# narayanan2004/GraphMat

Hardware: AMD Instinct MI355X
Metric: GTEPS (edges/s) per iter + achieved HBM GB/s, PageRank RMAT-26 (higher is better)
Workload: dtype f32

## Files before the change

graphmat_amd/csrc/gm_programs.hip:

```cpp
#include <limits.h>
#include <math.h>

#include <string>

#include "GraphMatRuntime.h"
#include "gm_internal.hpp"

#define HD __host__ __device__

namespace gm {

extern int g_short_row, g_giant_row, g_rank_by, g_rank_cap, g_col_tiles, g_tile_min_row, g_long_mid, g_tile_balance, g_own_wave_row, g_sort_tile_lists, g_sweep_slices, g_sweep_acc_limit, g_sweep_long_limit, g_sweep_long_row, g_sweep_fold_share, g_sweep_border_factor, g_blocked_rows, g_sweep_waves, g_sweep_stream, g_sweep_stream_weight;
static int g_force_ordered = 0;

struct PRv : gm_pr_t {
  HD PRv() { pagerank = 0.3; degree = 0; }
  HD int operator!=(const PRv& p) { return ((double)fabsf(p.pagerank - pagerank) > 1e-5); }
};

struct DegreeP : GraphMat::GraphProgram<int, int, PRv, int> {
  DegreeP() {
    this->order = GraphMat::IN_EDGES;
    this->process_message_requires_vertexprop = false;
  }
// ... 600 lines not shown

void warm_program_kernels(void* d_scratch256) {
  static bool done = false;
  if (done || !d_scratch256) return;
  done = true;
  hipLaunchKernelGGL(GraphMat::dev::k_fill_u32, dim3(1), dim3(GraphMat::dev::kBlock), 0, 0, (uint32_t*)d_scratch256, (int64_t)64, 0u);
  (void)hipDeviceSynchronize();
}

}

extern "C" {

namespace gm {
struct EngineKey { const char* name; int index; int def, lo, hi; };
static const EngineKey kEngineKeys[] = {
  {"debug_flags", 0, 0, 0, 0x7fffffff},
  {"wave16_form", 1, 2, 0, 31},
  {"rowwave_form", 2, 4, 0, 31},
  {"persist_per_cu", 3, 0, 0, 8},
  {"giant_maps", 4, 1, 0, 1},
  {"ordered_giant_two_pass", 5, 2, 0, 2},
  {"fuse_apply_send", 6, 1, 0, 1},
  {"untiled_pass_plain", 7, 1, 0, 1},
  {"last_rows_lanes", 8, 8, 8, 16},
  {"push_edge_permille", 9, 50, 0, 1000},
  {"bits_step_edges", 10, 2 << 20, 0, 0x7fffffff},
  {"sparse_step_edges", 11, 1 << 20, 0, 0x7fffffff},
  {"iteration_trace", 12, 0, 0, 1},
  {"ablate_cold_from", 13, 0, 0, 0x7fffffff},
  {"ablate_cold_short", 14, 0, 0, 0x7fffffff},
  {"two_stage_head_permille", 15, 900, 100, 990},
  {"giant_stream", 16, 1, 0, 2},
  {"sweep_form", 17, 0, 0, 511},
  {"blocked_form", 18, 2, 0, 31},
  {"guided_pull", 19, 1, 0, 2},
};
static_assert(offsetof(gm_engine_options_t, guided_pull) == 19 * sizeof(int32_t), "kEngineKeys follows the field order");
static bool engine_value_ok(const EngineKey& k, int v) {
  if (v < k.lo || v > k.hi) return false;
#ifndef GRAPHMAT_ABLATION
  if (!strcmp(k.name, "debug_flags") && (v & (15 | 16384)) != 0) return false;
  if (!strncmp(k.name, "ablate_", 7)) return false;
#endif
  if (!strcmp(k.name, "wave16_form")) return (v & 15) <= 5;
  if (!strcmp(k.name, "rowwave_form")) return (v & 15) <= 4;
  if (!strcmp(k.name, "last_rows_lanes")) return v == 8 || v == 16;
  return true;
}
static gm_engine_options_t engine_documented_defaults() {
  gm_engine_options_t o;
  memset(&o, 0, sizeof(o));
  for (const EngineKey& k : kEngineKeys) ((int32_t*)&o)[k.index] = k.def;
  const char* tr = getenv("GRAPHMAT_ITERATION_TRACE");
  if (tr && tr[0] == '1') o.iteration_trace = 1;
  if (const char* env = getenv("GRAPHMAT_OPTIONS")) {
    std::string all(env);
    size_t pos = 0;
    while (pos < all.size()) {
      size_t end = all.find(',', pos);
      if (end == std::string::npos) end = all.size();
      const std::string kv = all.substr(pos, end - pos);
      pos = end + 1;
      const size_t eq = kv.find('=');
      bool ok = false;
      if (eq != std::string::npos) {
        const std::string key = kv.substr(0, eq);
// ... 193 lines not shown
```

include/graphmat/engine.hpp:

```cpp
#pragma once
#include <stdio.h>
#include <stdlib.h>
#include <sys/time.h>

#include <limits>
#include <type_traits>
#include <vector>

#include "kernels.hpp"

namespace GraphMat {

enum edge_direction { OUT_EDGES, IN_EDGES, ALL_EDGES };
enum activity_type { ACTIVE_ONLY, ALL_VERTICES };

template <class T, class U, class V, class E>
class GraphProgram;

namespace detail {

template <class F>
struct member_class_of;
template <class C, class R, class... A>
struct member_class_of<R (C::*)(A...)> { typedef C type; };
// ... 784 lines not shown
        list_ready = frontier_v <= (unsigned long long)dev::kSparseListCap;
      }
    }
    if (xsparse_candidate) {
      int still = xsparse_ok ? 1 : 0;
      gm_graph_exchange(g, GM_XCHG_CONVERGED, nullptr, 0, nullptr, &still);
      if (!still) xsparse_ok = false;
    }
    if (xsparse_ok) {
      int dummy = 0;
      exchange_state(&dummy);
    }
    if (act == ALL_VERTICES) fill_active();
    timer = PhaseTimer(gm_graph_timing_enabled(g) != 0, s);
    tick("first frontier counted", (int)frontier_v);
    if (!(opt.debug_flags & dev::DBG_NO_OVERLAP)) {
      aux.attach(res_stream, res_fork, res_join);
    }
    if constexpr (program_row_filter<P>::enabled) {
      void* pw = nullptr;
      if (gm_graph_workspace(g, 8, ((size_t)(n + 31) / 32 + 2) * 4, &pw) == GM_OK) {
        d_want = (uint32_t*)pw;
        dev::ProgArg<P> pa0 = dev::make_prog_arg(gp);
        hipLaunchKernelGGL((dev::k_want_init<P, V>), dim3(grid_for(n_live)), dim3(dev::kBlock), 0, s, pa0, (const V*)d_vp, n_live, d_want);
      }
    }
    grouped_waves = !(opt.debug_flags & dev::DBG_NO_GROUPED);
  }

  void finish(int it) {
    GM_HIP_OK(hipStreamSynchronize(s));
    gm_graph_note_set(g, 3, (int64_t)sparse_sweeps);
    gm_graph_note_set(g, 4, (int64_t)short_folds);
    tick("loop done", it);
    aux.finish();
    st.iterations = it;
    timer.finish(&st);
    gm_graph_record_stats(g, &st);
    tick("teardown done", 0);
  }

  bool two_stage_applies() const {
    if (!(multi && act == ALL_VERTICES && order == OUT_EDGES && iterations > 0 && !(opt.debug_flags & dev::DBG_NO_PIPELINE) && !trace && inherits_iteration_hook<P>()))
      return false;
    if constexpr (sizeof(T) == 4 && sizeof(U) == 4 && std::is_trivially_copyable<T>::value && std::is_trivially_copyable<U>::value) {
      gm_sweep_t sw;
      if (!use_vp && gm_graph_sweep(g, &sw) == GM_OK && sw.nslices > 1 && desc.nshards > 1 && !(opt.debug_flags & (dev::DBG_NO_TILES | dev::DBG_NO_OVERLAP))) return false;
    }
    return true;
  }
  int run_two_stage() {
    void* x2v = nullptr;
    size_t x2_bytes = 0;
    int x2_ext = 0;
    int32_t rs = 0, bs = 0, ms = 0;
    bool staged = false;
    bool have_x2 = gm_graph_workspace_info(g, 9, &x2v, &x2_bytes, &x2_ext) == GM_OK && x2_ext && x2v != nullptr && x2_bytes >= (size_t)desc.ndevice * sizeof(T);
    if (!have_x2 && gm_graph_exchange_is_native(g))
      have_x2 = gm_graph_workspace(g, 9, (size_t)desc.ndevice * sizeof(T) + 64, &x2v) == GM_OK && x2v != nullptr;
    if (have_x2) {
      int64_t agreed = 0;
      if (gm_graph_note_get(g, 0, &agreed) == GM_OK) {
        rs = (int32_t)agreed;
        staged = rs > 0 && gm_graph_split(g, GM_DIR_OUT, opt.two_stage_head_permille, &rs, &bs, &ms) == GM_OK;
      } else {
        int mine = (gm_graph_split(g, GM_DIR_OUT, opt.two_stage_head_permille, &rs, &bs, &ms) == GM_OK) ? -rs : 0;
// ... 352 lines not shown
            hipLaunchKernelGGL((dev::k_spmv_sell_w12<P, T, U, V, E, false>), dim3(256), dim3(768), 0, s, pa, set, stage, sw.nslices, sw.nrows_long, sw.slice_base, sw.scol,
                               (const uint32_t*)nullptr, sw.wrow, sw.row_of_slot, sw.lcol, (const uint32_t*)nullptr, sw.lps, sw.lrow_of_slot, sw.gcol,
                               (const uint32_t*)nullptr, sw.gdst, sw.gslice, gt, xq, y);
          continue;
        }
        if (sterms != nullptr && set == 0) {
          if constexpr (sizeof(E) == 4 && std::is_trivially_copyable<E>::value) {
            if (Aout.vals != nullptr) {
              hipLaunchKernelGGL((dev::k_spmv_sell_stream<P, T, U, V, E, true>), dim3(256), dim3(1024), 0, s, pa, set, stage, sw.nslices, sw.nrows_long, sw.slice_base, sw.scol,
                                 sw.sval, sw.wrow_stream, sw.row_of_slot, sw.lcol, sw.lval, sw.lps, sw.lrow_of_slot, sw.gcol, sw.gval, sw.gdst, sw.gslice, gt, xq, y, sterms);
              with_vals = true;
            }
          }
          if (!with_vals)
            hipLaunchKernelGGL((dev::k_spmv_sell_stream<P, T, U, V, E, false>), dim3(256), dim3(1024), 0, s, pa, set, stage, sw.nslices, sw.nrows_long, sw.slice_base, sw.scol,
                               (const uint32_t*)nullptr, sw.wrow_stream, sw.row_of_slot, sw.lcol, (const uint32_t*)nullptr, sw.lps, sw.lrow_of_slot, sw.gcol,
                               (const uint32_t*)nullptr, sw.gdst, sw.gslice, gt, xq, y, sterms);
          continue;
        }
        if constexpr (sizeof(E) == 4 && std::is_trivially_copyable<E>::value) {
          if (Aout.vals != nullptr) {
            hipLaunchKernelGGL((dev::k_spmv_sell<P, T, U, V, E, true>), dim3(256), dim3(1024), 0, s, pa, set, stage, sw.nslices, sw.nrows_long, sw.slice_base, sw.scol,
                               sw.sval, sw.wrow, sw.row_of_slot, sw.lcol, sw.lval, sw.lps, sw.lrow_of_slot, sw.gcol, sw.gval, sw.gdst, sw.gslice, gt, xq, y);
            with_vals = true;
          }
        }
        if (!with_vals)
          hipLaunchKernelGGL((dev::k_spmv_sell<P, T, U, V, E, false>), dim3(256), dim3(1024), 0, s, pa, set, stage, sw.nslices, sw.nrows_long, sw.slice_base, sw.scol,
                             (const uint32_t*)nullptr, sw.wrow, sw.row_of_slot, sw.lcol, (const uint32_t*)nullptr, sw.lps, sw.lrow_of_slot, sw.gcol,
                             (const uint32_t*)nullptr, sw.gdst, sw.gslice, gt, xq, y);
      }
      st.spmv_launches += sw.nsets;
      timer.mark(TAG_WAVE);
      if (gterms != nullptr && !chain_done) {
        GM_HIP_OK(hipEventRecord(aux.fork, s));
        GM_HIP_OK(hipStreamWaitEvent(aux.s, aux.fork, 0));
        if (gather_apart) giant_gather();
        Launch Lg = L;
        Lg.terms_ready = true;
        launch_spmv_vp<P, T, U, V, E>(use_vp, Lg, pa, Ag, xq, xb, (const V*)d_vp, y, ybits, acc, rk);
      }
      if (where == 2) short_rows();
      if (where == 4) {
        hipLaunchKernelGGL((dev::k_short_fold<P, U>), dim3((unsigned)sw.nbins), dim3(512), 0, s, pa, (const U*)sterms, sw.sinv, sw.schunk, sw.nslices, sw.bin_cap, sw.sbin_row,
                           sw.soff, sw.srow, y, (acc & dev::ACC_STATIC_BITS) ? (uint32_t*)nullptr : ybits);
        st.spmv_launches++;
        short_folds++;
        if (verbose && !said_short_fold) { printf("GraphMat(HIP):   the rows of up to %d edges ride the sweep (k_short_fold)\n", (int)sw.short_row); said_short_fold = true; }
        timer.mark(TAG_ROWBLOCK);
      }
      if (aux.pending && !defer_join) GM_HIP_OK(hipStreamWaitEvent(s, aux.join, 0));
      aux.keep = aux.forked = aux.pending = false;
      timer.mark(defer_join ? TAG_ROWBLOCK : TAG_GIANT);
      if (shorts_blocked) {
        launch_blocked(pa, bl);
        st.spmv_launches += 1;
        timer.mark(TAG_ROWBLOCK);
      }
      if (!defer_join) check_probed(pa, Aout, xb != nullptr ? (const uint32_t*)ybits : Aout.rowbits, nullptr, acc, ybits, xb == nullptr);
    } else {
      (void)pa; (void)acc; (void)sw; (void)defer_join;
    }
  }

  bool swept_pipeline_applies(gm_sweep_t* sw) {
    if constexpr (kSparseT && sizeof(T) == 4 && sizeof(U) == 4 && std::is_trivially_copyable<U>::value) {
      if (!(multi && act == ALL_VERTICES && order == OUT_EDGES && iterations > 1 && !(opt.debug_flags & dev::DBG_NO_PIPELINE) && !trace && inherits_iteration_hook<P>())) return false;
      if (!(gm_graph_exchange_caps(g) & GM_XCAP_SPARSE) || rk_unverified || opt.fuse_apply_send == 0) return false;
      xq = x;
      xb = nullptr;
      int fine = (sweep_usable(dev::ACC_STATIC_BITS, sw) && sw->nsub > 1 && Aout.ngiant <= dev::kSparseListCap && n_live >= 64) ? 1 : 0;
      gm_graph_exchange(g, GM_XCHG_CONVERGED, nullptr, 0, nullptr, &fine);
      return fine == 1;
    } else {
      (void)sw;
      return false;
    }
  }
  int run_swept_sharded(const gm_sweep_t& sw) {
    if constexpr (kSparseT && sizeof(T) == 4 && sizeof(U) == 4 && std::is_trivially_copyable<U>::value) {
      void* x2v = nullptr;
// ... 55 lines not shown
          timer.mark(TAG_SEND);
          aux.wait_join(s);
          timer.mark(TAG_GIANT);
          hipLaunchKernelGGL((dev::k_apply_send_list<P, T, U, V>), dim3(grid_for(cap)), dim3(dev::kBlock), 0, s, pa, (const U*)y, (const uint32_t*)bits_giant, d_vp, d_active,
                             Aout.giant_row, Aout.ngiant, d_changed, xnext, desc.row_lo, gather + (size_t)desc.shard * cap, cap);
          timer.mark(TAG_APPLY);
          int hf[2] = {cap, 0};
          if (gm_graph_exchange(g, GM_XCHG_GATHER, gather, (int64_t)sizeof(xentry_t), nullptr, hf) != 0) die("giant rows' message exchange failed");
          if (gm_graph_exchange(g, GM_XCHG_WAIT, xnext, (int64_t)sizeof(T), nullptr, nullptr) != 0) die("message exchange wait failed");
          const int64_t nall = (int64_t)desc.nshards * cap;
          hipLaunchKernelGGL((dev::k_unpack_frontier<T>), dim3(grid_for(nall)), dim3(dev::kBlock), 0, s, (const xentry_t*)gather, nall, xnext, xbits);
          timer.mark(TAG_SEND);
        } else {
          hipLaunchKernelGGL((dev::k_apply<P, U, V, false>), dim3(ag), dim3(dev::kBlock), 0, s, pa, (const U*)y, Aout.rowbits, d_vp, d_active, n_live, d_changed,
                             (const int64_t*)nullptr, (unsigned long long*)nullptr, (uint32_t*)nullptr, (int32_t*)nullptr, (unsigned int*)nullptr);
          timer.mark(TAG_APPLY);
        }
        if (n_live < n && it == 0) GM_HIP_OK(hipMemsetAsync(d_active + n_live / 32, 0, (size_t)(nwords - n_live / 32) * 4, s));
        gp->do_every_iteration(it);
        T* t = xcur; xcur = xnext; xnext = t;
      }
      fill_active();
      finish(it);
      return it;
    } else {
      (void)sw;
      return -1;
    }
  }

  bool said_blocked = false, said_sparse_sweep = false, said_short_fold = false;
  int sparse_sweeps = 0;
  int short_folds = 0;
  bool blocked_usable(int acc, gm_blocked_t* bl) {
    if constexpr (sizeof(T) == 4 && sizeof(U) == 4 && std::is_trivially_copyable<T>::value && std::is_trivially_copyable<U>::value) {
      if (use_vp || xq == nullptr || xb != nullptr || d_want != nullptr || program_row_filter<P>::enabled || (acc & dev::ACC_READ_PREV)) return false;
      if (!(rk == REDUCE_ORDERED || rk == REDUCE_F32_ADD || rk == REDUCE_COMMUTATIVE)) return false;
      if (opt.debug_flags & dev::DBG_NO_TILES) return false;
      if (gm_graph_blocked(g, bl) != GM_OK || bl->nrows <= 0 || bl->short_row != Aout.short_row) return false;
      if (Aout.vals != nullptr && !(bl->val_bytes == 4 && bl->eval != nullptr && sizeof(E) == 4 && std::is_trivially_copyable<E>::value)) return false;
      return true;
    } else {
      (void)acc; (void)bl;
      return false;
    }
  }
  void launch_blocked(const dev::ProgArg<P>& pa, const gm_blocked_t& bl) {
    if constexpr (sizeof(T) == 4 && sizeof(U) == 4 && std::is_trivially_copyable<T>::value && std::is_trivially_copyable<U>::value) {
      static int cus_of[64] = {0};
      constexpr bool kValsOk = sizeof(E) == 4 && std::is_trivially_copyable<E>::value;
      int dev_id = 0;
      GM_HIP_OK(hipGetDevice(&dev_id));
      int& cus = cus_of[dev_id & 63];
      if (cus == 0) {
        GM_HIP_OK(hipFuncSetAttribute((const void*)&dev::k_spmv_blocked<P, T, U, V, E, false, 2>, hipFuncAttributeMaxDynamicSharedMemorySize, GM_BLOCKED_ROWS * 4));
        GM_HIP_OK(hipFuncSetAttribute((const void*)&dev::k_spmv_blocked<P, T, U, V, E, false, 4>, hipFuncAttributeMaxDynamicSharedMemorySize, GM_BLOCKED_ROWS * 4));
        if constexpr (kValsOk) {
          GM_HIP_OK(hipFuncSetAttribute((const void*)&dev::k_spmv_blocked<P, T, U, V, E, true, 2>, hipFuncAttributeMaxDynamicSharedMemorySize, GM_BLOCKED_ROWS * 4));
          GM_HIP_OK(hipFuncSetAttribute((const void*)&dev::k_spmv_blocked<P, T, U, V, E, true, 4>, hipFuncAttributeMaxDynamicSharedMemorySize, GM_BLOCKED_ROWS * 4));
        }
        int n = 0;
        GM_HIP_OK(hipDeviceGetAttribute(&n, hipDeviceAttributeMultiprocessorCount, dev_id));
        cus = n > 0 ? n : 1;
      }
      if (verbose && !said_blocked) { printf("GraphMat(HIP):   the short rows take the column-blocked stream (%d rows, %lld edges%s)\n", bl.nrows, (long long)bl.nentries, Aout.vals ? ", with their edge values" : ""); said_blocked = true; }
      static int fits_of[64] = {0};
// ... 121 lines not shown
        const int nf = (int)frontier_v;
        const unsigned pieces = (unsigned)(frontier_e / dev::kPieceEdges + frontier_v);
        piece_offsets(nf);
        hipLaunchKernelGGL(dev::k_mark_rows_of_list, dim3(pieces > 0 ? pieces : 1), dim3(dev::kBlock), 0, s, Asrc, (const int32_t*)d_list, nf, (const unsigned int*)d_off, d_mark);
      } else {
        const int mgrid = grid_for(n_live) < 4096 ? grid_for(n_live) : 4096;
        hipLaunchKernelGGL(dev::k_mark_rows_of_active, dim3(mgrid), dim3(dev::kBlock), 0, s, Asrc, (const uint32_t*)d_active, n_live, d_mark);
      }
      row_bits = d_mark;
      guided_few = frontier_e <= 4096ull;
      if (verbose) printf("GraphMat(HIP):   guided pull: %llu active vertices, %llu out-edges\n", frontier_v, frontier_e);
    }
    if (dense_push) {
      multiply_dense_push(pa);
    } else if (order == OUT_EDGES || order == ALL_EDGES) {
      const int acc = static_bits ? dev::ACC_STATIC_BITS : 0;
      const uint32_t* xsum = nullptr;
      const unsigned long long present_x = xsparse_ok ? (unsigned long long)xs_total : frontier_v;
      if (want_stats && rk == REDUCE_LAST && xb != nullptr && present_x * 512ull < (unsigned long long)n_live * (unsigned long long)desc.nshards) {
        void* ps = nullptr;
        const int xwords = (desc.ndevice + 31) / 32;
        const int nsum = (xwords / 2 + 31) / 32 + 1;
        if (gm_graph_workspace(g, 11, (size_t)nsum * 4 + 64, &ps) == GM_OK) {
          hipLaunchKernelGGL(dev::k_bits_summary, dim3(grid_for(nsum)), dim3(dev::kBlock), 0, s, xb, xwords, (uint32_t*)ps, nsum);
          xsum = (const uint32_t*)ps;
        }
      }
      int ntile = 1;
      if (dense_x && !multi && row_bits == nullptr && rk != REDUCE_LAST && dev::stageable<T>::value && !(opt.debug_flags & dev::DBG_NO_TILES))
        gm_graph_tiles(g, GM_DIR_OUT, &ntile);
      gm_sweep_t sw;
      gm_blocked_t bl;
      if (row_bits == nullptr && !xsp && sweep_usable(acc, &sw)) {
        multiply_out_swept(pa, acc, sw);
      } else if (dense_x && !multi && row_bits == nullptr && blocked_usable(acc, &bl)) {
        multiply_out_blocked(pa, acc, bl);
      } else if (ntile > 1) {
        multiply_out_tiled(pa, ntile, acc);
      } else {
        launch_spmv_vp<P, T, U, V, E>(use_vp, launch_ctx(), pa, Aout, xq, xb, (const V*)d_vp, y, ybits, acc, rk, row_bits, grouped_waves && guided_few, xsum);
        check_probed(pa, Aout, static_bits ? Aout.rowbits : (const uint32_t*)ybits, row_bits, acc, ybits, dense_x);
      }
      if (static_bits) apply_bits = Aout.rowbits;
    }
    if (!dense_push && (order == IN_EDGES || order == ALL_EDGES)) {
      int acc = (order == ALL_EDGES) ? dev::ACC_READ_PREV : 0;
      uint32_t* yb = ybits;
      if (static_bits) {
        acc |= dev::ACC_STATIC_BITS;
        yb = const_cast<uint32_t*>(Aout.rowbits);
        apply_bits = Ain.rowbits;
        if (order == ALL_EDGES && gm_graph_rowbits_all(g, &apply_bits) != GM_OK) die(gm_last_error());
      }
      launch_spmv_vp<P, T, U, V, E>(use_vp, launch_ctx(), pa, Ain, (const T*)x, xb, (const V*)d_vp, y, yb, acc, rk, (const uint32_t*)d_want, grouped_waves);
      if (order == IN_EDGES) check_probed(pa, Ain, static_bits ? Ain.rowbits : (const uint32_t*)ybits, d_want, acc, ybits, dense_x);
    }
    lap("SPMV time");
    if (trace) tr_updated = count_bits(apply_bits, n_live);
    const bool build_list = want_stats && frontier_e <= (4ull << 20);
    if (want_stats) GM_HIP_OK(hipMemsetAsync(d_count, 0, 4, s));
    listed = build_list;
    const int apply_cap = build_list ? dev::kApplyMaxBlocks / 4 : dev::kApplyMaxBlocks;
    const int apply_grid = grid_for(n_live) < apply_cap ? grid_for(n_live) : apply_cap;
    if (want_stats)
      hipLaunchKernelGGL((dev::k_apply<P, U, V, true>), dim3(apply_grid), dim3(dev::kBlock), 0, s, pa, (const U*)y, apply_bits, d_vp, d_active, n_live,
                         d_changed, Asrc.rowptr, d_striped, d_want, build_list ? d_list : (int32_t*)nullptr, build_list ? d_count : (unsigned int*)nullptr);
    else if (inherits_iteration_hook<P>() && dense_x && !lazy_send && !trace && opt.fuse_apply_send != 0 && iterations > 0 && it + 1 < iterations) {
      hipLaunchKernelGGL((dev::k_apply_send<P, T, U, V>), dim3(apply_grid), dim3(dev::kBlock), 0, s, pa, (const U*)y, apply_bits, d_vp, d_active, n_live,
                         d_changed, d_want, x, xbits, desc.row_lo);
      x_presend = true;
    } else
      hipLaunchKernelGGL((dev::k_apply<P, U, V, false>), dim3(apply_grid), dim3(dev::kBlock), 0, s, pa, (const U*)y, apply_bits, d_vp, d_active, n_live,
                         d_changed, (const int64_t*)nullptr, (unsigned long long*)nullptr, d_want, (int32_t*)nullptr, (unsigned int*)nullptr);
    if (n_live < n && it == 0)
      GM_HIP_OK(hipMemsetAsync(d_active + n_live / 32, 0, (size_t)(nwords - n_live / 32) * 4, s));
    timer.mark(TAG_APPLY);
    lap("Apply time");
  }

  int run_loop() {
    int it = 0;
    tick("setup done", 0);
    while (true) {
      tick("iteration", it);
      if (trace) { (void)hipStreamSynchronize(s); gettimeofday(&tr_iter, 0); tr_last = tr_iter; }
      tr_updated = -1;
      if (verbose && can_push) printf("GraphMat(HIP):   active set: %llu vertices, %llu out-edges (max %llu)\n", frontier_v, frontier_e, frontier_maxdeg);
      dev::ProgArg<P> pa = dev::make_prog_arg(gp);
      const bool want_stats = (can_push || xsparse_ok || guided) && iterations <= 0;
      if (iterations <= 0) GM_HIP_OK(hipMemsetAsync(d_changed, 0, want_stats ? sizeof(int) + striped_bytes : sizeof(int), s));
      timer.mark(TAG_START);
      const bool xsp = xsparse_ok && xs_max <= dev::kSparseListCap &&
                       (unsigned long long)xs_max * sizeof(xentry_t) * 2ull < (unsigned long long)n_live * sizeof(T);
      const bool push = can_push && frontier_v > 0 && frontier_v <= (unsigned long long)dev::kSparseListCap &&
                        frontier_e * 1000ull < (unsigned long long)Aout.nnz * (unsigned long long)opt.push_edge_permille;
      const bool sparse = push && frontier_e <= (unsigned long long)opt.sparse_step_edges;
      const bool dense_push = push && !sparse && rk == REDUCE_LAST;
// ... 56 lines not shown
```

include/graphmat/kernels.hpp:

```cpp
#pragma once
#include <hip/hip_runtime.h>
#include <stdint.h>
#include <string.h>

#include <type_traits>

#include "../graphmat_hip.h"

namespace GraphMat {

enum reduce_kind {
  REDUCE_AUTO = -1,
  REDUCE_ORDERED = 0,
  REDUCE_COMMUTATIVE = 1,
  REDUCE_LAST = 2,
  REDUCE_F32_ADD = 3
};

template <class P>
struct program_traits {
  static constexpr reduce_kind reduce = REDUCE_AUTO;
};

template <class P>
// ... 1587 lines not shown
      if (row >= 0 && ((s_hasbits[i >> 5] >> (i & 31)) & 1u)) { y[row] = as_u(s_acc[i]); atomicOr(&ybits[row >> 5], 1u << (row & 31)); }
    } else {
      if (row >= 0) y[row] = as_u(s_acc[i]);
    }
  }
  if (lj >= 0 && nrows_long > 0) {
    const int row = lrow_of_slot[vw * NLP + lj];
    if (row >= 0 && lhas) {
      y[row] = lacc;
      if constexpr (SPARSE) atomicOr(&ybits[row >> 5], 1u << (row & 31));
    }
  }
}
template <class P, class T, class U, class V, class E, bool HAS_VALS, int ABL = 0, int UBATCH = 7, int PIPE = 2, int POOLW = GM_SWEEP_POOL>
__global__ void __launch_bounds__(1024)
k_spmv_sell(ProgArg<P> pa, int set, int stage_words, int nslices, int nrows_long, const int32_t* __restrict__ slice_base, const uint32_t* __restrict__ scol,
            const uint32_t* __restrict__ sval, const uint32_t* __restrict__ wrow, const int32_t* __restrict__ row_of_slot, const uint32_t* __restrict__ lcol,
            const uint32_t* __restrict__ lval, const uint32_t* __restrict__ lps, const int32_t* __restrict__ lrow_of_slot,
            const uint32_t* __restrict__ gcol, const uint32_t* __restrict__ gval, const uint32_t* __restrict__ gdst, const uint32_t* __restrict__ gslice,
            U* __restrict__ gterms, const T* __restrict__ x, U* __restrict__ y) {
  sell_body<P, T, U, V, E, HAS_VALS, ABL, UBATCH, PIPE, POOLW, false>(pa, set, stage_words, nslices, nrows_long, slice_base, scol, sval, wrow, row_of_slot, lcol, lval, lps,
                                                                       lrow_of_slot, gcol, gval, gdst, gslice, gterms, x, y, 1, 0, 0);
}
template <class P, class T, class U, class V, class E, bool HAS_VALS>
__global__ void __launch_bounds__(1024)
k_spmv_sell_stream(ProgArg<P> pa, int set, int stage_words, int nslices, int nrows_long, const int32_t* __restrict__ slice_base, const uint32_t* __restrict__ scol,
                   const uint32_t* __restrict__ sval, const uint32_t* __restrict__ wrow, const int32_t* __restrict__ row_of_slot, const uint32_t* __restrict__ lcol,
                   const uint32_t* __restrict__ lval, const uint32_t* __restrict__ lps, const int32_t* __restrict__ lrow_of_slot,
                   const uint32_t* __restrict__ gcol, const uint32_t* __restrict__ gval, const uint32_t* __restrict__ gdst, const uint32_t* __restrict__ gslice,
                   U* __restrict__ gterms, const T* __restrict__ x, U* __restrict__ y, U* __restrict__ sterms) {
  sell_body<P, T, U, V, E, HAS_VALS, 0, 7, 2, GM_SWEEP_POOL, false>(pa, set, stage_words, nslices, nrows_long, slice_base, scol, sval, wrow, row_of_slot, lcol, lval, lps,
                                                                     lrow_of_slot, gcol, gval, gdst, gslice, gterms, x, y, 1, 0, 0, nullptr, nullptr, sterms);
}
template <class P, class U>
__global__ void __launch_bounds__(512, 6)
k_short_fold(ProgArg<P> pa, const U* __restrict__ sterms, const uint16_t* __restrict__ sinv, const uint32_t* __restrict__ schunk, int nslices, int cap,
             const uint32_t* __restrict__ sbin_row, const uint32_t* __restrict__ soff, const int32_t* __restrict__ srow_id, U* __restrict__ y,
             uint32_t* __restrict__ ybits) {
  static_assert(sizeof(U) == 4, "4-byte reductions");
  __shared__ uint32_t s_prod[(GM_STREAM_BIN + 64) + (GM_STREAM_BIN + 64) / 32 + 1];
  auto at = [](uint32_t q) { return q + (q >> 5); };
  __shared__ uint32_t s_cpos[GM_MAX_SLICES], s_cpre[GM_MAX_SLICES + 1];
  const P& p = *reinterpret_cast<const P*>(pa.b);
  const int b = blockIdx.x, wv = threadIdx.x >> 6, lane = threadIdx.x & 63;
  const uint32_t* __restrict__ raw = reinterpret_cast<const uint32_t*>(sterms);
  const uint32_t i0 = sbin_row[b], i1 = sbin_row[b + 1], base = (uint32_t)b * (uint32_t)cap;
  constexpr int RK = 4;
  uint32_t ro0[RK], ro1[RK];
  int rid[RK];
#pragma unroll
  for (int j = 0; j < RK; j++) {
    const uint32_t i = i0 + (uint32_t)(j * 512) + threadIdx.x;
    if (i < i1) { ro0[j] = soff[i]; ro1[j] = soff[i + 1]; rid[j] = srow_id[i]; }
  }
  if ((int)threadIdx.x < nslices) {
    const uint2 pn = *reinterpret_cast<const uint2*>(&schunk[((size_t)b * nslices + threadIdx.x) * 2]);
    s_cpos[threadIdx.x] = pn.x;
    s_cpre[threadIdx.x] = pn.y;
  }
  __syncthreads();
  constexpr int CB = 4, CK = 4;
  for (int c0 = wv; c0 < nslices; c0 += 8 * CB) {
    uint32_t vv[CB][CK];
    uint16_t qq[CB][CK];
    uint32_t cp[CB], cn[CB];
#pragma unroll
    for (int c = 0; c < CB; c++) {
      const int sl = c0 + 8 * c;
      cp[c] = sl < nslices ? s_cpos[sl] : 0u;
      cn[c] = sl < nslices ? s_cpre[sl] : 0u;
    }
#pragma unroll
    for (int c = 0; c < CB; c++) {
#pragma unroll
      for (int k = 0; k < CK; k++) {
        const uint32_t i = (uint32_t)(k * 64 + lane);
        if (i < cn[c]) {
          vv[c][k] = __builtin_nontemporal_load(&raw[cp[c] + i]);
          qq[c][k] = __builtin_nontemporal_load(&sinv[cp[c] + i]);
        }
      }
    }
#pragma unroll
    for (int c = 0; c < CB; c++) {
#pragma unroll
      for (int k = 0; k < CK; k++)
        if ((uint32_t)(k * 64 + lane) < cn[c]) s_prod[at(qq[c][k])] = vv[c][k];
      for (uint32_t i = (uint32_t)(CK * 64 + lane); i < cn[c]; i += 64u) s_prod[at(sinv[cp[c] + i])] = raw[cp[c] + i];
    }
  }
  __syncthreads();
  auto as_u = [](uint32_t r) { U u; __builtin_memcpy(&u, &r, 4); return u; };
  for (uint32_t ii = i0 + (uint32_t)(wv * 64), jj = 0; ii < i1; ii += 512u, jj++) {
    const uint32_t i = ii + (uint32_t)lane;
    const bool valid = i < i1;
    int row = 0;
    if (valid) {
      uint32_t o0, o1;
      if (jj < RK) {
        o0 = ro0[0]; o1 = ro1[0]; row = rid[0];
#pragma unroll
        for (int j = 1; j < RK; j++) if ((int)jj == j) { o0 = ro0[j]; o1 = ro1[j]; row = rid[j]; }
      } else { o0 = soff[i]; o1 = soff[i + 1]; row = srow_id[i]; }
      o0 -= base; o1 -= base;
      U acc = as_u(s_prod[at(o0)]);
      for (uint32_t k = o0 + 1; k < o1; k++) p.P::reduce_function(acc, as_u(s_prod[at(k)]));
      y[row] = acc;
    }
    if (ybits != nullptr) {
      const int r0 = __builtin_amdgcn_readfirstlane(row);
      if (__all(!valid || row == r0 + lane)) {
        const unsigned long long hb = __ballot(valid);
        const int sh = r0 & 31;
        const unsigned long long lo = hb << sh, hi = sh ? (hb >> (64 - sh)) : 0ull;
        const uint32_t w = lane == 0 ? (uint32_t)lo : lane == 1 ? (uint32_t)(lo >> 32) : lane == 2 ? (uint32_t)hi : 0u;
        if (lane < 3 && w != 0u) atomicOr(&ybits[(r0 >> 5) + lane], w);
      } else if (valid) {
        atomicOr(&ybits[row >> 5], 1u << (row & 31));
      }
    }
  }
}
template <class P, class T, class U, class V, class E, bool HAS_VALS>
__global__ void __launch_bounds__(kBlock)
k_giant_gather_sliced(ProgArg<P> pa, const uint32_t* __restrict__ gcol, const uint32_t* __restrict__ gval, const uint32_t* __restrict__ gdst, int64_t n,
                      const T* __restrict__ x, U* __restrict__ gterms) {
  static_assert(sizeof(T) == 4 && sizeof(U) == 4, "4-byte messages and reductions");
  const P& p = *reinterpret_cast<const P*>(pa.b);
  V no_vp;
  for (int64_t i = (int64_t)blockIdx.x * kBlock + threadIdx.x; i < n; i += (int64_t)gridDim.x * kBlock) {
    const uint32_t c4 = __builtin_nontemporal_load(&gcol[i]), d = __builtin_nontemporal_load(&gdst[i]);
    E ev = E();
    if constexpr (HAS_VALS) { const uint32_t raw = __builtin_nontemporal_load(&gval[i]); __builtin_memcpy(&ev, &raw, 4); }
    const T m = *reinterpret_cast<const T*>(reinterpret_cast<const char*>(x) + c4);
    U res;
    p.P::process_message(m, ev, no_vp, res);
    gterms[d] = res;
  }
}

template <class P, class T, class U, class V, class E, bool HAS_VALS>
__global__ void __launch_bounds__(768)
k_spmv_sell_w12(ProgArg<P> pa, int set, int stage_words, int nslices, int nrows_long, const int32_t* __restrict__ slice_base, const uint32_t* __restrict__ scol,
                const uint32_t* __restrict__ sval, const uint32_t* __restrict__ wrow, const int32_t* __restrict__ row_of_slot, const uint32_t* __restrict__ lcol,
                const uint32_t* __restrict__ lval, const uint32_t* __restrict__ lps, const int32_t* __restrict__ lrow_of_slot,
                const uint32_t* __restrict__ gcol, const uint32_t* __restrict__ gval, const uint32_t* __restrict__ gdst, const uint32_t* __restrict__ gslice,
                U* __restrict__ gterms, const T* __restrict__ x, U* __restrict__ y) {
  sell_body<P, T, U, V, E, HAS_VALS, 0, 7, 2, GM_SWEEP_POOL_W12, false, 768>(pa, set, stage_words, nslices, nrows_long, slice_base, scol, sval, wrow, row_of_slot, lcol, lval, lps,
                                                                             lrow_of_slot, gcol, gval, gdst, gslice, gterms, x, y, 1, 0, 0);
}

template <class P, class T, class U, class V, class E, bool HAS_VALS>
__global__ void __launch_bounds__(1024)
// ... 1551 lines not shown
```

Before: 329.5.

## Fuse apply and send into the short-row fold and per-row tail kernels

When the sweep path folds short rows, the fold kernel now applies the vertex program and writes the next message directly, and a side-stream kernel applies the long and giant rows from their slot lists. This skips the separate full-vertex apply/send pass and the y/ybits round trip for those rows. It adds gating conditions, a second stream dependency, and risks missing rows that appear in neither list. A test app checks correctness, and setting bit 512 of sweep_form disables the fusion.

```diff
diff --git a/apps/fused_tail_hooks.cpp b/apps/fused_tail_hooks.cpp
--- /dev/null
+++ b/apps/fused_tail_hooks.cpp
@@ -0,0 +1,112 @@
+#include <cstdio>
+#include <cstdlib>
+#include <vector>
+
+#include "GraphMatRuntime.h"
+
+static int failures = 0;
+#define CHECK(cond)                                                    \
+  do {                                                                 \
+    if (!(cond)) { printf("CHECK failed: %s (line %d)\n", #cond, __LINE__); failures++; } \
+  } while (0)
+
+class Plain : public GraphMat::GraphProgram<float, float, float> {
+ public:
+  float gain;
+  Plain() : gain(2.0f) { this->process_message_requires_vertexprop = false; this->activity = GraphMat::ALL_VERTICES; }
+  bool send_message(const float& v, float& m) const { m = v * gain; return true; }
+  void process_message(const float& m, const int e, const float&, float& r) const { r = m * (float)e; }
+  void reduce_function(float& a, const float& b) const { a += b; }
+  void apply(const float& y, float& v) { v = (float)((long long)y % 97 + 1); }
+};
+class Hooked : public Plain {
+ public:
+  void do_every_iteration(int) {}
+};
+class EveryTime : public Plain {
+ public:
+  void do_every_iteration(int it) { gain = (float)(it % 6 + 3); }
+};
+
+namespace GraphMat {
+template <> struct program_traits<Plain> { static constexpr reduce_kind reduce = REDUCE_F32_ADD; };
+template <> struct program_traits<Hooked> { static constexpr reduce_kind reduce = REDUCE_F32_ADD; };
+template <> struct program_traits<EveryTime> { static constexpr reduce_kind reduce = REDUCE_F32_ADD; };
+}
+
+typedef std::vector<GraphMat::edge_t<int> > edges_t;
+
+template <class PROG>
+static bool run_and_compare(GraphMat::Graph<float>& G, const edges_t& ed, int n, int iters, long long want_note) {
+  std::vector<float> v(n + 1), y(n + 1);
+  std::vector<char> has(n + 1);
+  for (int u = 1; u <= n; u++) v[u] = (float)(u % 97 + 1);
+  for (int u = 1; u <= n; u++) G.setVertexproperty(u, v[u]);
+  PROG host;
+  for (int it = 0; it < iters; it++) {
+    std::fill(y.begin(), y.end(), 0.0f);
+    std::fill(has.begin(), has.end(), 0);
+    for (auto& e : ed) {
+      float m, r;
+      host.send_message(v[e.src], m);
+      host.process_message(m, e.val, 0.0f, r);
+      y[e.dst] += r;
+      has[e.dst] = 1;
+    }
+    for (int u = 1; u <= n; u++)
+      if (has[u]) host.apply(y[u], v[u]);
+    host.do_every_iteration(it);
+  }
+  PROG prog;
+  G.setAllActive();
+  GraphMat::run_graph_program(&prog, G, iters);
+  bool ok = true;
+  int shown = 0;
+  for (int u = 1; u <= n; u++) {
+    const float got = G.getVertexproperty(u);
+    if (got != v[u]) {
+      ok = false;
+      if (shown++ < 3) printf("  vertex %d: %.1f, expected %.1f\n", u, got, v[u]);
+    }
+  }
+  int64_t folds = -1, tails = -1;
+  CHECK(gm_graph_note_get(G.A, 4, &folds) == 0 && folds == iters);
+  CHECK(gm_graph_note_get(G.A, 5, &tails) == 0);
+  if (tails != want_note) { printf("  fused tails: %lld, expected %lld\n", (long long)tails, want_note); ok = false; }
+  return ok;
+}
+
+int main(int argc, char** argv) {
+  MPI_Init(&argc, &argv);
+  setenv("GRAPHMAT_COL_TILES", "4", 1);
+  CHECK(gm_set_option("sweep_form", 256) == 0);
+  const int n = 6000;
+  edges_t ed;
+  unsigned st = 4321u;
+  auto next = [&]() { st = st * 1664525u + 1013904223u; return st >> 8; };
+  for (int h = 0; h < 24; h++)
+    for (int k = 0; k < (h == 0 ? 6000 : h <= 3 ? 1200 + 300 * h : 70 + 7 * h); k++) ed.push_back(GraphMat::edge_t<int>(1 + (int)(next() % n), 1 + h, 1 + (int)(next() % 3)));
+  for (int i = 0; i < n; i += 2) ed.push_back(GraphMat::edge_t<int>(1 + i, 1 + (i + 1) % n, 2));
+  for (int i = 0; i < 3 * n; i++) ed.push_back(GraphMat::edge_t<int>(1 + (int)(next() % n), 1 + (int)(next() % n), 1 + (int)(next() % 3)));
+  GraphMat::Graph<float> G;
+  GraphMat::edgelist_t<int> E(n, n, (int)ed.size());
+  std::copy(ed.begin(), ed.end(), E.edges);
+  G.ReadEdgelist(E);
+  E.clear();
+  gm_sweep_t sw;
+  gm_csr_t ca;
+  CHECK(gm_graph_sweep(G.A, &sw) == 0 && gm_graph_csr(G.A, GM_DIR_OUT, &ca) == 0);
+  printf("sweep: %d rows (%d long), %lld short-row edges in its stream, %d giant rows\n", sw.nrows, sw.nrows_long, (long long)sw.nstream, ca.ngiant);
+  CHECK(sw.nrows > sw.nrows_long && sw.nrows_long > 0 && sw.nstream > 0 && ca.ngiant > 0);
+  for (int iters = 1; iters <= 5; iters += 2) {
+    const bool a = run_and_compare<Plain>(G, ed, n, iters, iters), b = run_and_compare<Hooked>(G, ed, n, iters, 0), c = run_and_compare<EveryTime>(G, ed, n, iters, 0);
+    CHECK(gm_set_option("sweep_form", 256 | 512) == 0);
+    const bool d = run_and_compare<Plain>(G, ed, n, iters, 0);
+    CHECK(gm_set_option("sweep_form", 256) == 0);
+    printf("%d iterations: plain %s, hooked %s, every-time %s, plain with the separate pass %s\n", iters, a ? "ok" : "WRONG", b ? "ok" : "WRONG", c ? "ok" : "WRONG", d ? "ok" : "WRONG");
+    CHECK(a); CHECK(b); CHECK(c); CHECK(d);
+  }
+  printf(failures == 0 ? "FUSEDTAIL PASS\n" : "FUSEDTAIL FAIL (%d)\n", failures);
+  MPI_Finalize();
+  return failures == 0 ? 0 : 1;
+}
diff --git a/graphmat_amd/csrc/gm_programs.hip b/graphmat_amd/csrc/gm_programs.hip
--- a/graphmat_amd/csrc/gm_programs.hip
+++ b/graphmat_amd/csrc/gm_programs.hip
@@ -656,7 +656,7 @@
   {"ablate_cold_short", 14, 0, 0, 0x7fffffff},
   {"two_stage_head_permille", 15, 900, 100, 990},
   {"giant_stream", 16, 1, 0, 2},
-  {"sweep_form", 17, 0, 0, 511},
+  {"sweep_form", 17, 0, 0, 1023},
   {"blocked_form", 18, 2, 0, 31},
   {"guided_pull", 19, 1, 0, 2},
 };
diff --git a/include/graphmat/engine.hpp b/include/graphmat/engine.hpp
--- a/include/graphmat/engine.hpp
+++ b/include/graphmat/engine.hpp
@@ -840,6 +840,7 @@
     GM_HIP_OK(hipStreamSynchronize(s));
     gm_graph_note_set(g, 3, (int64_t)sparse_sweeps);
     gm_graph_note_set(g, 4, (int64_t)short_folds);
+    gm_graph_note_set(g, 5, (int64_t)fused_tails);
     tick("loop done", it);
     aux.finish();
     st.iterations = it;
@@ -1258,21 +1259,51 @@
       }
       st.spmv_launches += sw.nsets;
       timer.mark(TAG_WAVE);
-      if (gterms != nullptr && !chain_done) {
+      const int tail = (tail_want != 0 && where == 4 && sw.nsub <= 1 && !multi && !defer_join && (acc & dev::ACC_STATIC_BITS) && xb == nullptr &&
+                        ((gterms != nullptr && !gather_apart && !chain_done) || Aout.ngiant == 0)) ? tail_want : 0;
+      auto apply_rows = [&](const int32_t* la, int na, const int32_t* lb, int nb) {
+        if (na + nb <= 0) return;
+        if (tail == 1)
+          hipLaunchKernelGGL((dev::k_apply_rows<P, T, U, V, true>), dim3(grid_for(na + nb)), dim3(dev::kBlock), 0, aux.s, pa, (const U*)y, d_vp, la, na, lb, nb, x, desc.row_lo);
+        else
+          hipLaunchKernelGGL((dev::k_apply_rows<P, T, U, V, false>), dim3(grid_for(na + nb)), dim3(dev::kBlock), 0, aux.s, pa, (const U*)y, d_vp, la, na, lb, nb, x, desc.row_lo);
+      };
+      if ((gterms != nullptr && !chain_done) || tail) {
         GM_HIP_OK(hipEventRecord(aux.fork, s));
         GM_HIP_OK(hipStreamWaitEvent(aux.s, aux.fork, 0));
-        if (gather_apart) giant_gather();
-        Launch Lg = L;
-        Lg.terms_ready = true;
-        launch_spmv_vp<P, T, U, V, E>(use_vp, Lg, pa, Ag, xq, xb, (const V*)d_vp, y, ybits, acc, rk);
+        if (gterms != nullptr) {
+          if (gather_apart) giant_gather();
+          Launch Lg = L;
+          Lg.terms_ready = true;
+          launch_spmv_vp<P, T, U, V, E>(use_vp, Lg, pa, Ag, xq, xb, (const V*)d_vp, y, ybits, acc, rk);
+        }
+        if (tail) {
+          apply_rows(sw.row_of_slot, sw.nsets * 256 * GM_SWEEP_ACC_ROWS, sw.nrows_long > 0 ? sw.lrow_of_slot : (const int32_t*)nullptr,
+                     sw.nrows_long > 0 ? sw.nsets * 256 * GM_SWEEP_LONG_SLOTS : 0);
+          apply_rows(Aout.giant_row, gterms != nullptr ? Aout.ngiant : 0, (const int32_t*)nullptr, 0);
+          GM_HIP_OK(hipEventRecord(aux.join, aux.s));
+          aux.pending = true;
+        }
       }
       if (where == 2) short_rows();
       if (where == 4) {
-        hipLaunchKernelGGL((dev::k_short_fold<P, U>), dim3((unsigned)sw.nbins), dim3(512), 0, s, pa, (const U*)sterms, sw.sinv, sw.schunk, sw.nslices, sw.bin_cap, sw.sbin_row,
-                           sw.soff, sw.srow, y, (acc & dev::ACC_STATIC_BITS) ? (uint32_t*)nullptr : ybits);
+        if (tail == 1)
+          hipLaunchKernelGGL((dev::k_short_fold_apply<P, T, U, V, true>), dim3((unsigned)sw.nbins), dim3(512), 0, s, pa, (const U*)sterms, sw.sinv, sw.schunk, sw.nslices, sw.bin_cap,
+                             sw.sbin_row, sw.soff, sw.srow, d_vp, x, desc.row_lo);
+        else if (tail == 2)
+          hipLaunchKernelGGL((dev::k_short_fold_apply<P, T, U, V, false>), dim3((unsigned)sw.nbins), dim3(512), 0, s, pa, (const U*)sterms, sw.sinv, sw.schunk, sw.nslices, sw.bin_cap,
+                             sw.sbin_row, sw.soff, sw.srow, d_vp, x, desc.row_lo);
+        else
+          hipLaunchKernelGGL((dev::k_short_fold<P, U>), dim3((unsigned)sw.nbins), dim3(512), 0, s, pa, (const U*)sterms, sw.sinv, sw.schunk, sw.nslices, sw.bin_cap, sw.sbin_row,
+                             sw.soff, sw.srow, y, (acc & dev::ACC_STATIC_BITS) ? (uint32_t*)nullptr : ybits);
         st.spmv_launches++;
         short_folds++;
         if (verbose && !said_short_fold) { printf("GraphMat(HIP):   the rows of up to %d edges ride the sweep (k_short_fold)\n", (int)sw.short_row); said_short_fold = true; }
+        if (tail) {
+          tail_taken = true;
+          fused_tails++;
+          if (verbose && !said_fused_tail) { printf("GraphMat(HIP):   fused tail: the rows are applied where they are folded (k_short_fold_apply, k_apply_rows)\n"); said_fused_tail = true; }
+        }
         timer.mark(TAG_ROWBLOCK);
       }
       if (aux.pending && !defer_join) GM_HIP_OK(hipStreamWaitEvent(s, aux.join, 0));
@@ -1394,6 +1425,9 @@
   bool said_blocked = false, said_sparse_sweep = false, said_short_fold = false;
   int sparse_sweeps = 0;
   int short_folds = 0;
+  int tail_want = 0;
+  bool tail_taken = false, said_fused_tail = false;
+  int fused_tails = 0;
   bool blocked_usable(int acc, gm_blocked_t* bl) {
     if constexpr (sizeof(T) == 4 && sizeof(U) == 4 && std::is_trivially_copyable<T>::value && std::is_trivially_copyable<U>::value) {
       if (use_vp || xq == nullptr || xb != nullptr || d_want != nullptr || program_row_filter<P>::enabled || (acc & dev::ACC_READ_PREV)) return false;
@@ -1581,7 +1615,11 @@
       gm_sweep_t sw;
       gm_blocked_t bl;
       if (row_bits == nullptr && !xsp && sweep_usable(acc, &sw)) {
+        if (order == OUT_EDGES && static_bits && dense_x && !multi && !want_stats && inherits_iteration_hook<P>() && !lazy_send && !trace && opt.fuse_apply_send != 0 &&
+            iterations > 0 && !rk_unverified && d_want == nullptr && !(opt.sweep_form & 512))
+          tail_want = it + 1 < iterations ? 1 : 2;
         multiply_out_swept(pa, acc, sw);
+        tail_want = 0;
       } else if (dense_x && !multi && row_bits == nullptr && blocked_usable(acc, &bl)) {
         multiply_out_blocked(pa, acc, bl);
       } else if (ntile > 1) {
@@ -1611,7 +1649,10 @@
     listed = build_list;
     const int apply_cap = build_list ? dev::kApplyMaxBlocks / 4 : dev::kApplyMaxBlocks;
     const int apply_grid = grid_for(n_live) < apply_cap ? grid_for(n_live) : apply_cap;
-    if (want_stats)
+    if (tail_taken) {
+      tail_taken = false;
+      x_presend = it + 1 < iterations;
+    } else if (want_stats)
       hipLaunchKernelGGL((dev::k_apply<P, U, V, true>), dim3(apply_grid), dim3(dev::kBlock), 0, s, pa, (const U*)y, apply_bits, d_vp, d_active, n_live,
                          d_changed, Asrc.rowptr, d_striped, d_want, build_list ? d_list : (int32_t*)nullptr, build_list ? d_count : (unsigned int*)nullptr);
     else if (inherits_iteration_hook<P>() && dense_x && !lazy_send && !trace && opt.fuse_apply_send != 0 && iterations > 0 && it + 1 < iterations) {
diff --git a/include/graphmat/kernels.hpp b/include/graphmat/kernels.hpp
--- a/include/graphmat/kernels.hpp
+++ b/include/graphmat/kernels.hpp
@@ -1643,11 +1643,11 @@
   sell_body<P, T, U, V, E, HAS_VALS, 0, 7, 2, GM_SWEEP_POOL, false>(pa, set, stage_words, nslices, nrows_long, slice_base, scol, sval, wrow, row_of_slot, lcol, lval, lps,
                                                                      lrow_of_slot, gcol, gval, gdst, gslice, gterms, x, y, 1, 0, 0, nullptr, nullptr, sterms);
 }
-template <class P, class U>
-__global__ void __launch_bounds__(512, 6)
-k_short_fold(ProgArg<P> pa, const U* __restrict__ sterms, const uint16_t* __restrict__ sinv, const uint32_t* __restrict__ schunk, int nslices, int cap,
-             const uint32_t* __restrict__ sbin_row, const uint32_t* __restrict__ soff, const int32_t* __restrict__ srow_id, U* __restrict__ y,
-             uint32_t* __restrict__ ybits) {
+template <class P, class U, int TAIL, class T, class V>
+__device__ __forceinline__ void
+short_fold_body(const ProgArg<P>& pa, const U* __restrict__ sterms, const uint16_t* __restrict__ sinv, const uint32_t* __restrict__ schunk, int nslices, int cap,
+                const uint32_t* __restrict__ sbin_row, const uint32_t* __restrict__ soff, const int32_t* __restrict__ srow_id, U* __restrict__ y,
+                uint32_t* __restrict__ ybits, V* __restrict__ vp, T* __restrict__ x, int row_base) {
   static_assert(sizeof(U) == 4, "4-byte reductions");
   __shared__ uint32_t s_prod[(GM_STREAM_BIN + 64) + (GM_STREAM_BIN + 64) / 32 + 1];
   auto at = [](uint32_t q) { return q + (q >> 5); };
@@ -1714,10 +1714,26 @@
         for (int j = 1; j < RK; j++) if ((int)jj == j) { o0 = ro0[j]; o1 = ro1[j]; row = rid[j]; }
       } else { o0 = soff[i]; o1 = soff[i + 1]; row = srow_id[i]; }
       o0 -= base; o1 -= base;
-      U acc = as_u(s_prod[at(o0)]);
-      for (uint32_t k = o0 + 1; k < o1; k++) p.P::reduce_function(acc, as_u(s_prod[at(k)]));
-      y[row] = acc;
-    }
+      if constexpr (TAIL != 0) {
+        V cur = vp[row];
+        U acc = as_u(s_prod[at(o0)]);
+        for (uint32_t k = o0 + 1; k < o1; k++) p.P::reduce_function(acc, as_u(s_prod[at(k)]));
+        ProgArg<P> local = pa;
+        P& pl = *reinterpret_cast<P*>(local.b);
+        pl.P::apply(acc, cur);
+        vp[row] = cur;
+        if constexpr (TAIL == 1) {
+          T m;
+          p.P::send_message(cur, m);
+          x[(size_t)row_base + row] = m;
+        }
+      } else {
+        U acc = as_u(s_prod[at(o0)]);
+        for (uint32_t k = o0 + 1; k < o1; k++) p.P::reduce_function(acc, as_u(s_prod[at(k)]));
+        y[row] = acc;
+      }
+    }
+    if constexpr (TAIL != 0) continue;
     if (ybits != nullptr) {
       const int r0 = __builtin_amdgcn_readfirstlane(row);
       if (__all(!valid || row == r0 + lane)) {
@@ -1730,6 +1746,40 @@
         atomicOr(&ybits[row >> 5], 1u << (row & 31));
       }
     }
+  }
+}
+template <class P, class U>
+__global__ void __launch_bounds__(512, 6)
+k_short_fold(ProgArg<P> pa, const U* __restrict__ sterms, const uint16_t* __restrict__ sinv, const uint32_t* __restrict__ schunk, int nslices, int cap,
+             const uint32_t* __restrict__ sbin_row, const uint32_t* __restrict__ soff, const int32_t* __restrict__ srow_id, U* __restrict__ y,
+             uint32_t* __restrict__ ybits) {
+  short_fold_body<P, U, 0, U, int>(pa, sterms, sinv, schunk, nslices, cap, sbin_row, soff, srow_id, y, ybits, (int*)nullptr, (U*)nullptr, 0);
+}
+template <class P, class T, class U, class V, bool SEND>
+__global__ void __launch_bounds__(512, 6)
+k_short_fold_apply(ProgArg<P> pa, const U* __restrict__ sterms, const uint16_t* __restrict__ sinv, const uint32_t* __restrict__ schunk, int nslices, int cap,
+                   const uint32_t* __restrict__ sbin_row, const uint32_t* __restrict__ soff, const int32_t* __restrict__ srow_id, V* __restrict__ vp,
+                   T* __restrict__ x, int row_base) {
+  short_fold_body<P, U, SEND ? 1 : 2, T, V>(pa, sterms, sinv, schunk, nslices, cap, sbin_row, soff, srow_id, (U*)nullptr, (uint32_t*)nullptr, vp, x, row_base);
+}
+template <class P, class T, class U, class V, bool SEND>
+__global__ void __launch_bounds__(kBlock)
+k_apply_rows(ProgArg<P> pa, const U* __restrict__ y, V* __restrict__ vp, const int32_t* __restrict__ list_a, int na, const int32_t* __restrict__ list_b, int nb,
+             T* __restrict__ x, int row_base) {
+  const int i = blockIdx.x * kBlock + threadIdx.x;
+  if (i >= na + nb) return;
+  const int r = i < na ? list_a[i] : list_b[i - na];
+  if (r < 0) return;
+  ProgArg<P> local = pa;
+  P& p = *reinterpret_cast<P*>(local.b);
+  V cur = vp[r];
+  p.P::apply(y[r], cur);
+  vp[r] = cur;
+  if constexpr (SEND) {
+    const P& ps = *reinterpret_cast<const P*>(pa.b);
+    T m;
+    ps.P::send_message(cur, m);
+    x[(size_t)row_base + r] = m;
   }
 }
 template <class P, class T, class U, class V, class E, bool HAS_VALS>
```

Measured after the change: 321.7. -2.4%, worse.
